# SreenivasVRao/SuperSloMo-VideoInterpolation-PyTorch

Measured on AMD Instinct MI355X. Metric: interpolated 1280x720 frames/sec, higher is better.
Workload: dtype f32

## Files before the change

superslomo-videointerpolation-pytorch_amd/csrc/ssm_wino5.hip:

```cpp
#include "ssm_common.h"
#include "ssm_wino5_pack.h"

#include <atomic>
#include <mutex>
#include <type_traits>
#include <cstdlib>

typedef float f32x4 __attribute__((ext_vector_type(4)));
typedef float f32x2 __attribute__((ext_vector_type(2)));

namespace {

struct W5Params {
    const float *src;
    long long sb, sc;
    int sh;
    int Cin;
    const float *wpk;
    const float *bias;
    float *dst;
    long long dsb, dsc;
    int dsh;
    float *pool;
    long long psb, psc;
    int psh;
    int H, W, Cout;
    int tilesX, tilesY, NB;
    float slope;
    int lrelu;
    int vec;
    const float *add;
    long long asb, asc;
    int ash, adiv;
    unsigned long long *dbg;
};

template <int GTX_, int WTY_, int WTX_>
struct W5Cfg {
    static constexpr int GTX = GTX_, GTY = 16 / GTX_, WTY = WTY_, WTX = WTX_;
    static constexpr int NTX = GTX * WTX, NTY = GTY * WTY, NT = 32;
    static constexpr int TH = 4 * NTY, TW = 4 * NTX;
    static constexpr int CK = 4;
    static constexpr int PH = TH + 4, PW = TW + 8;
    static constexpr int SHIFT = 2;
    static constexpr int NFQ = 16;
    static constexpr int USZ = NFQ * CK * 32 * 4;
    static constexpr int NTP = NT + 2;
    static constexpr int XRW = NTX * 4 + 4;
    static constexpr int VSZ = NFQ * CK * NTP * 4;
    static constexpr int XPL = PH * XRW;
    static constexpr int XSZ = CK * 2 * XPL;
    static constexpr int NDQ = CK * PH * PW / 4, NGP = (NDQ + 63) / 64;
    static constexpr int PCAP = NGP * 256 + 256;
    static constexpr int NGU = USZ / 256, NIU = NGU / 4, NIP = (NGP + 3) / 4;
    static constexpr int NRU = PH * NTX, NRR = (NRU + 63) / 64;
    static constexpr int UOFF = 0, VOFF = 2 * USZ, XOFF = VOFF + VSZ, POFF = XOFF + XSZ;
    static constexpr int BYTES = (POFF + 2 * PCAP) * 4;
    static_assert(WTY * WTX == 2 && (GTX == 4 || GTX == 8 || GTX == 16), "two tile groups of 16 tiles");
    static_assert(PW % 4 == 0 && NGU % 4 == 0, "whole DMA groups");
    static_assert(BYTES <= 160 * 1024, "LDS budget");
};

__device__ __forceinline__ void w5_bt(const float (&e)[8], float (&f)[8]) {
    f[0] = (e[0] - e[6]) + 5.25f * (e[4] - e[2]);
    f[7] = (e[7] - e[1]) + 5.25f * (e[3] - e[5]);
    const float t1 = (e[2] + e[6]) - 4.25f * e[4], t2 = (e[1] + e[5]) - 4.25f * e[3];
    const float t3 = (e[6] + 0.25f * e[2]) - 1.25f * e[4], t4 = (0.5f * e[1] - 2.5f * e[3]) + 2.f * e[5];
    const float t5 = (e[6] + 4.f * e[2]) - 5.f * e[4], t6 = (2.f * e[1] - 2.5f * e[3]) + 0.5f * e[5];
    f[1] = t1 + t2;
    f[2] = t1 - t2;
    f[3] = t3 + t4;
    f[4] = t3 - t4;
    f[5] = t5 + t6;
    f[6] = t5 - t6;
}

__device__ __forceinline__ void w5_at(float m0, float m1, float m2, float m3, float m4, float m5, float m6, float m7, float (&y)[4]) {
    const float s1 = m1 + m2, t1 = m1 - m2, s2 = m3 + m4, t2 = m3 - m4, s3 = m5 + m6, t3 = m5 - m6;
    y[0] = (m0 + s1) + (s2 + s3);
    y[1] = (t1 + 2.f * t2) + 0.5f * t3;
    y[2] = (s1 + 4.f * s2) + 0.25f * s3;
    y[3] = ((t1 + 8.f * t2) + 0.125f * t3) + m7;
}

template <bool FAST>
__device__ __forceinline__ void w5_epilogue(const W5Params &p, const f32x4 (&acc)[64], const float (&bv)[4], int b, int cu0, int q, int px, int py) {
    const float sl = (p.lrelu & 1) ? p.slope : 1.f;
    const bool amask = (p.lrelu & 2) != 0;
    float *dstb = p.dst + (long long)b * p.dsb;
    float *poolb = p.pool ? p.pool + (long long)b * p.psb : nullptr;
    const unsigned pb = 4u * ((unsigned)(4 * q) * (unsigned)p.dsc + (unsigned)py * (unsigned)p.dsh + (unsigned)px);
    const unsigned qb = 4u * ((unsigned)(4 * q) * (unsigned)p.psc + (unsigned)(py >> 1) * (unsigned)p.psh + (unsigned)(px >> 1));
    const bool vok = FAST || (py + 4 <= p.H && px + 4 <= p.W && p.vec);
    auto st4 = [](const float *base, unsigned off_bytes, f32x4 val) {
        asm volatile("global_store_dwordx4 %0, %1, %2" ::"v"(off_bytes), "v"(val), "s"(base) : "memory");
    };
    auto st2 = [](const float *base, unsigned off_bytes, f32x2 val) {
        asm volatile("global_store_dwordx2 %0, %1, %2" ::"v"(off_bytes), "v"(val), "s"(base) : "memory");
    };
    auto st1 = [](const float *base, unsigned off_bytes, float val) {
        asm volatile("global_store_dword %0, %1, %2" ::"v"(off_bytes), "v"(val), "s"(base) : "memory");
    };
    const float *addb = p.add ? p.add + (long long)(b / p.adiv) * p.asb + (long long)(4 * q) * p.asc + (long long)py * p.ash + px : nullptr;
    f32x4 zadd[2][4];
    const bool zvec = p.add && vok;
    auto zload = [&](int r) {
        if (zvec) {
#pragma unroll
            for (int i = 0; i < 4; ++i) zadd[r & 1][i] = *(const f32x4 *)(addb + (long long)(cu0 + r) * p.asc + (long long)i * p.ash);
        }
    };
    zload(0);
#pragma unroll
    for (int r = 0; r < 4; ++r) {
        const int cu = cu0 + r;
        if (r + 1 < 4) zload(r + 1);
        float t[4][8];
#pragma unroll
        for (int cf = 0; cf < 8; ++cf) {
            float y4[4];
            w5_at(acc[cf][r], acc[8 + cf][r], acc[16 + cf][r], acc[24 + cf][r], acc[32 + cf][r], acc[40 + cf][r], acc[48 + cf][r], acc[56 + cf][r], y4);
#pragma unroll
            for (int i = 0; i < 4; ++i) t[i][cf] = y4[i];
        }
        float y[4][4];
#pragma unroll
        for (int i = 0; i < 4; ++i) {
            float y4[4];
            w5_at(t[i][0], t[i][1], t[i][2], t[i][3], t[i][4], t[i][5], t[i][6], t[i][7], y4);
#pragma unroll
            for (int e = 0; e < 4; ++e) y[i][e] = y4[e] + bv[r];
        }
        if (p.add) {
            const float *ap = addb + (long long)cu * p.asc;
#pragma unroll
            for (int i = 0; i < 4; ++i) {
                if (vok) {
                    const f32x4 z = zadd[r & 1][i];
                    if (amask) {
#pragma unroll
                        for (int e = 0; e < 4; ++e) y[i][e] *= z[e] > 0.f ? 1.f : p.slope;
                    } else {
                        y[i][0] += z[0];
                        y[i][1] += z[1];
                        y[i][2] += z[2];
                        y[i][3] += z[3];
                    }
                } else {
#pragma unroll
                    for (int e = 0; e < 4; ++e)
                        if (py + i < p.H && px + e < p.W) {
                                const float z = ap[(long long)i * p.ash + e];
                                y[i][e] = amask ? y[i][e] * (z > 0.f ? 1.f : p.slope) : y[i][e] + z;
                            }
                }
            }
        }
#pragma unroll
        for (int i = 0; i < 4; ++i)
#pragma unroll
            for (int e = 0; e < 4; ++e) y[i][e] = fmaxf(y[i][e], y[i][e] * sl);
        if (zvec && r + 1 < 4) {
#pragma unroll
            for (int i = 0; i < 4; ++i) asm volatile("" : "+v"(zadd[(r + 1) & 1][i]));
        }
        float *bp = dstb + (long long)cu * p.dsc;
#pragma unroll
        for (int i = 0; i < 4; ++i) {
            if (vok) {
                st4(bp + (long long)i * p.dsh, pb, f32x4{y[i][0], y[i][1], y[i][2], y[i][3]});
            } else {
#pragma unroll
                for (int e = 0; e < 4; ++e)
                    if (py + i < p.H && px + e < p.W) st1(bp + (long long)i * p.dsh + e, pb, y[i][e]);
            }
        }
        if (poolb) {
            float *qp = poolb + (long long)cu * p.psc;
#pragma unroll
            for (int i = 0; i < 2; ++i) {
                const float o0 = ((y[2 * i][0] + y[2 * i + 1][0]) + (y[2 * i][1] + y[2 * i + 1][1])) * 0.25f;
                const float o1 = ((y[2 * i][2] + y[2 * i + 1][2]) + (y[2 * i][3] + y[2 * i + 1][3])) * 0.25f;
                const bool rok = FAST || py + 2 * i < p.H;
                if (FAST || (rok && px + 4 <= p.W && p.vec)) st2(qp + (long long)i * p.psh, qb, f32x2{o0, o1});
                else if (rok) {
                    if (px + 2 <= p.W) st1(qp + (long long)i * p.psh, qb, o0);
                    if (px + 4 <= p.W) st1(qp + (long long)i * p.psh + 1, qb, o1);
                }
            }
        }
        __builtin_amdgcn_sched_barrier(0);
    }
}

#if !W5_SPLIT
template <class C>
__global__ __launch_bounds__(256) __attribute__((amdgpu_waves_per_eu(1, 1))) void wino5_kernel(const W5Params p) {
    extern __shared__ __attribute__((aligned(16))) float lds[];
    constexpr int PH = C::PH, PW = C::PW, NTX = C::NTX, CK = C::CK, NFQ = C::NFQ;

    const int tid = threadIdx.x;
    const int lane = tid & 63, l15 = lane & 15, q = lane >> 4;
    const int wid = __builtin_amdgcn_readfirstlane(tid >> 6);
    const int cb = wid & 1, tg = wid >> 1;

    int id = ssm_xcd_tile(blockIdx.x, gridDim.x);
    const int nb = id % p.NB;
    id /= p.NB;
    const int tx = id % p.tilesX;
    id /= p.tilesX;
    const int ty = id % p.tilesY;
    const int b = id / p.tilesY;
    const int x0 = tx * C::TW, y0 = ty * C::TH;

    const float *pbase = p.src + (long long)b * p.sb + (long long)(y0 - 2) * p.sh + (x0 - 4);
    const float *wbase = p.wpk + (long long)nb * (p.Cin / CK) * C::USZ;

    int poff[C::NIP];
#pragma unroll
    for (int i = 0; i < C::NIP; ++i) {
        const int qq = (i * 4 + wid) * 64 + lane;
        if (qq < C::NDQ) {
            const int c = qq / (PH * (PW / 4)), rem = qq - c * (PH * (PW / 4));
            const int r = rem / (PW / 4), j = rem - r * (PW / 4);
            const int re = min(r, p.H + (SSM_PADY - 1) - (y0 - 2)), fe = min(4 * j, ((p.W + 2 * SSM_PADX + 3) & ~3) - 4 - x0);
            poff[i] = ((int)(c * p.sc) + re * p.sh + fe) * 4;
        } else {
            poff[i] = 0;
        }
    }
    const int uoff = lane * 16;
    const unsigned lds0 = (unsigned)(size_t)(__attribute__((address_space(3))) void *)lds;
    auto dma = [](const float *base, int voff_bytes, unsigned m0v) {
        asm volatile("s_mov_b32 m0, %2\n\ts_nop 0\n\tglobal_load_lds_dwordx4 %0, %1" ::"v"(voff_bytes), "s"(base), "s"(m0v) : "memory", "m0");
    };
    auto issue_n = [&](int s, int n) {
        const int buf = s & 1;
        if (n < C::NIP) {
            const int g = 4 * n + wid;
            if (4 * n + 3 < C::NGP || g < C::NGP) {
                const float *base = pbase + (long long)(s * CK) * p.sc;
                const unsigned m0v = __builtin_amdgcn_readfirstlane(lds0 + (unsigned)(C::POFF + buf * C::PCAP + C::SHIFT) * 4u + (unsigned)g * 1024u);
                dma(base, poff[n], m0v);
            }
        } else {
            const int g = 4 * (n - C::NIP) + wid;
            const float *base = wbase + (long long)s * C::USZ + g * 256;
            const unsigned m0v = __builtin_amdgcn_readfirstlane(lds0 + (unsigned)(C::UOFF + buf * C::USZ) * 4u + (unsigned)g * 1024u);
            dma(base, uoff, m0v);
        }
    };
    static_assert(C::NIP + C::NIU <= 16, "one DMA slot per quad of the matrix phase");

    f32x4 acc[64];
#pragma unroll
    for (int f = 0; f < 64; ++f) acc[f] = f32x4{0.f, 0.f, 0.f, 0.f};
    float bv[4];
#pragma unroll
    for (int r = 0; r < 4; ++r) bv[r] = p.bias[nb * 32 + cb * 16 + 4 * q + r];

    int r_src[C::NRR], r_dst[C::NRR];
#pragma unroll
    for (int k = 0; k < C::NRR; ++k) {
        const int u = min(lane + 64 * k, C::NRU - 1);
        const int c = wid, row = u / NTX, t = u - row * NTX;
        r_src[k] = C::POFF + C::SHIFT + (c * PH + row) * PW + 4 * t + 2;
        r_dst[k] = C::XOFF + c * 2 * C::XPL + row * C::XRW + t * 4;
    }
    const int c_tile = lane & 31;
    const int c_gx = (c_tile & 15) % C::GTX, c_gy = (c_tile & 15) / C::GTX, c_g2 = c_tile >> 4;
    const int c_Tx = (c_g2 % C::WTX) * C::GTX + c_gx, c_Ty = (c_g2 / C::WTX) * C::GTY + c_gy;
    const int c_src = C::XOFF + (wid * 2 + (lane >> 5)) * C::XPL + (4 * c_Ty) * C::XRW + c_Tx * 4;
    const int c_dst = C::VOFF + (((lane >> 5) * CK + wid) * C::NTP + c_tile) * 4;

    const f32x4 *lds4 = (const f32x4 *)lds;
    const int aBase = C::UOFF / 4 + q * 32 + cb * 16 + l15;
    const int bBase = C::VOFF / 4 + q * C::NTP + tg * 16 + l15;
    const int gx = l15 % C::GTX, gy = l15 / C::GTX;
    const int Tx = (tg % C::WTX) * C::GTX + gx, Ty = (tg / C::WTX) * C::GTY + gy;

    const int nsteps = p.Cin / CK;
#pragma unroll
    for (int n = 0; n < C::NIP + C::NIU; ++n) issue_n(0, n);
#ifdef W5_TRACE
    unsigned long long tph[6] = {0, 0, 0, 0, 0, 0};
    unsigned long long tk = __builtin_amdgcn_s_memtime();
    const unsigned long long tstart = tk;
#define W5STAMP(i)                                                  \
    {                                                               \
        const unsigned long long tn = __builtin_amdgcn_s_memtime(); \
        tph[i] += tn - tk;                                          \
        tk = tn;                                                    \
    }
#else
#define W5STAMP(i)
#endif
    for (int s = 0; s < nsteps; ++s) {
        const bool more = s + 1 < nsteps;
        W5STAMP(3)
        asm volatile("s_waitcnt vmcnt(0)" ::: "memory");
        __syncthreads();
        W5STAMP(0)
        {
            f32x4 ra[C::NRR][2];
#pragma unroll
            for (int k = 0; k < C::NRR; ++k) {
                const float *src = lds + r_src[k] + (s & 1) * C::PCAP;
                ra[k][0] = *(const f32x4 *)src;
                ra[k][1] = *(const f32x4 *)(src + 4);
            }
#pragma unroll
            for (int k = 0; k < C::NRR; ++k) {
                const float e[8] = {ra[k][0][0], ra[k][0][1], ra[k][0][2], ra[k][0][3], ra[k][1][0], ra[k][1][1], ra[k][1][2], ra[k][1][3]};
                float f[8];
                w5_bt(e, f);
                float *dst = lds + r_dst[k];
                *(f32x4 *)dst = f32x4{f[0], f[1], f[2], f[3]};
                *(f32x4 *)(dst + C::XPL) = f32x4{f[4], f[5], f[6], f[7]};
            }
        }
        W5STAMP(1)
        __builtin_amdgcn_wave_barrier();
        W5STAMP(4)
        {
            f32x4 cx[8];
#pragma unroll
            for (int i = 0; i < 8; ++i) cx[i] = *(const f32x4 *)(lds + c_src + i * C::XRW);
            float f[4][8];
#pragma unroll
            for (int e = 0; e < 4; ++e) {
                float d[8] = {cx[0][e], cx[1][e], cx[2][e], cx[3][e], cx[4][e], cx[5][e], cx[6][e], cx[7][e]};
#pragma unroll
                for (int i = 0; i < 8; ++i) asm volatile("" : "+v"(d[i]));
                w5_bt(d, f[e]);
            }
#pragma unroll
            for (int rf = 0; rf < 8; ++rf) *(f32x4 *)(lds + c_dst + rf * 2 * CK * C::NTP * 4) = f32x4{f[0][rf], f[1][rf], f[2][rf], f[3][rf]};
        }
        W5STAMP(2)
        __syncthreads();
        W5STAMP(5)
        {
            const int ai = aBase + (s & 1) * (C::USZ / 4), bi = bBase;
            f32x4 a[3], bq[3];
            a[0] = lds4[ai];
            bq[0] = lds4[bi];
            a[1] = lds4[ai + CK * 32];
            bq[1] = lds4[bi + CK * C::NTP];
#pragma unroll
            for (int g = 0; g < NFQ; ++g) {
                const int cur = g % 3, nxt = (g + 2) % 3;
#pragma unroll
                for (int e = 0; e < 4; ++e) {
                    acc[4 * g + e] = __builtin_amdgcn_mfma_f32_16x16x4f32(a[cur][e], bq[cur][e], acc[4 * g + e], 0, 0, 0);
                    if (e == 0) {
                        __builtin_amdgcn_sched_barrier(0);
                        if (g + 2 < NFQ) {
                            a[nxt] = lds4[ai + (g + 2) * CK * 32];
                            bq[nxt] = lds4[bi + (g + 2) * CK * C::NTP];
                        }
                        __builtin_amdgcn_sched_barrier(0);
                    }
                    if (e == 1 && g < C::NIP + C::NIU && more) {
                        issue_n(s + 1, g);
                        __builtin_amdgcn_sched_barrier(0);
                    }
                }
                __builtin_amdgcn_sched_barrier(0);
            }
        }
    }
    W5STAMP(3)
    {
        const int px = x0 + 4 * Tx, py = y0 + 4 * Ty;
        w5_epilogue<false>(p, acc, bv, b, nb * 32 + cb * 16, q, px, py);
    }
#ifdef W5_TRACE
    asm volatile("s_waitcnt vmcnt(0)" ::: "memory");
    if (p.dbg && lane == 0 && (blockIdx.x % 64) == 0) {
        const unsigned long long tn = __builtin_amdgcn_s_memtime();
        for (int i = 0; i < 6; ++i) atomicAdd(p.dbg + wid * 8 + i, tph[i]);
        atomicAdd(p.dbg + wid * 8 + 6, tn - tk);
        atomicAdd(p.dbg + wid * 8 + 7, 1ULL);
        (void)tstart;
    }
#endif
}

#endif

#if W5_SPLIT
__device__ __forceinline__ void w5_bt_lo(const float (&e)[8], float (&f)[4]) {
    f[0] = (e[0] - e[6]) + 5.25f * (e[4] - e[2]);
    f[3] = (e[7] - e[1]) + 5.25f * (e[3] - e[5]);
    const float t1 = (e[2] + e[6]) - 4.25f * e[4], t2 = (e[1] + e[5]) - 4.25f * e[3];
    f[1] = t1 + t2;
    f[2] = t1 - t2;
}
__device__ __forceinline__ void w5_bt_hi(const float (&e)[8], float (&f)[4]) {
    const float t3 = (e[6] + 0.25f * e[2]) - 1.25f * e[4], t4 = (0.5f * e[1] - 2.5f * e[3]) + 2.f * e[5];
    const float t5 = (e[6] + 4.f * e[2]) - 5.f * e[4], t6 = (2.f * e[1] - 2.5f * e[3]) + 0.5f * e[5];
    f[0] = t3 + t4;
    f[1] = t3 - t4;
    f[2] = t5 + t6;
    f[3] = t5 - t6;
}

template <class C>
struct W5SLds {
    static constexpr int NPB = 3;
    static constexpr int XRW = C::NTX * 4 + 8, XPL = C::PH * XRW;
    static constexpr int XSZ1 = C::CK * XPL;
    static constexpr int UOFF = 0, VOFF = 2 * C::USZ, XOFF = VOFF + C::VSZ, POFF = XOFF + XSZ1;
    static constexpr int BYTES = (POFF + NPB * C::PCAP) * 4;
    static constexpr int EXSZ = 8 * 2 * 4 * 64 * 4;
    static_assert(BYTES <= 160 * 1024 && EXSZ <= 2 * C::USZ, "LDS budget; the exchange area reuses the filter stages");
};

template <class C>
__global__ __launch_bounds__(512) __attribute__((amdgpu_waves_per_eu(2, 2))) void wino5s_kernel(const W5Params p) {
    extern __shared__ __attribute__((aligned(16))) float lds[];
    using L = W5SLds<C>;
    constexpr int PH = C::PH, PW = C::PW, NTX = C::NTX, CK = C::CK, NTP = C::NTP;

    const int tid = threadIdx.x;
    const int lane = tid & 63, l15 = lane & 15, q = lane >> 4;
    const int wid = __builtin_amdgcn_readfirstlane(tid >> 6);
    const int cb = wid & 1, tg = (wid >> 1) & 1, fh = wid >> 2;
    const int w4 = wid & 3;

    int id = ssm_xcd_tile(blockIdx.x, gridDim.x);
    const int nb = id % p.NB;
    id /= p.NB;
    const int tx = id % p.tilesX;
    id /= p.tilesX;
    const int ty = id % p.tilesY;
    const int b = id / p.tilesY;
    const int x0 = tx * C::TW, y0 = ty * C::TH;

    const float *pbase = p.src + (long long)b * p.sb + (long long)(y0 - 2) * p.sh + (x0 - 4);
    const float *wbase = p.wpk + (long long)nb * (p.Cin / CK) * C::USZ;

    int poff[C::NIP];
#pragma unroll
    for (int i = 0; i < C::NIP; ++i) {
        const int qq = (i * 4 + w4) * 64 + lane;
        if (qq < C::NDQ) {
            const int c = qq / (PH * (PW / 4)), rem = qq - c * (PH * (PW / 4));
            const int r = rem / (PW / 4), j = rem - r * (PW / 4);
            const int re = min(r, p.H + (SSM_PADY - 1) - (y0 - 2)), fe = min(4 * j, ((p.W + 2 * SSM_PADX + 3) & ~3) - 4 - x0);
            poff[i] = ((int)(c * p.sc) + re * p.sh + fe) * 4;
        } else {
            poff[i] = 0;
        }
    }
    const int uoff = lane * 16;
    const unsigned lds0 = (unsigned)(size_t)(__attribute__((address_space(3))) void *)lds;
    auto dma = [](const float *base, int voff_bytes, unsigned m0v) {
        asm volatile("s_mov_b32 m0, %2\n\ts_nop 0\n\tglobal_load_lds_dwordx4 %0, %1" ::"v"(voff_bytes), "s"(base), "s"(m0v) : "memory", "m0");
    };
    struct DmaBase {
        const float *src;
        unsigned m0;
    };
    auto u_base = [&](int s) {
        return DmaBase{wbase + (long long)s * C::USZ + w4 * 256,
                       (unsigned)__builtin_amdgcn_readfirstlane(lds0 + (unsigned)(L::UOFF + (s & 1) * C::USZ) * 4u + (unsigned)w4 * 1024u)};
    };
    auto p_base = [&](int s, int pb) {
        return DmaBase{pbase + (long long)(s * CK) * p.sc,
                       (unsigned)__builtin_amdgcn_readfirstlane(lds0 + (unsigned)(L::POFF + pb * C::PCAP + C::SHIFT) * 4u + (unsigned)w4 * 1024u)};
    };
    auto dma_u = [&](const DmaBase &bs, int k) { dma(bs.src + k * 1024, uoff, bs.m0 + (unsigned)k * 4096u); };
    auto dma_p = [&](const DmaBase &bs, int k) {
        if (4 * k + 3 < C::NGP || 4 * k + w4 < C::NGP) dma(bs.src, poff[k], bs.m0 + (unsigned)k * 4096u);
    };
    static_assert(C::NGU == 32, "8 filter pieces per wave of half 1: the transform's 8 DMA slots");

    f32x4 acc[32];
#pragma unroll
    for (int f = 0; f < 32; ++f) acc[f] = f32x4{0.f, 0.f, 0.f, 0.f};

    int r_src[C::NRR], r_dst[C::NRR];
#pragma unroll
    for (int k = 0; k < C::NRR; ++k) {
        const int u = min(lane + 64 * k, C::NRU - 1);
        const int row = u / NTX, t = u - row * NTX;
        r_src[k] = L::POFF + C::SHIFT + (w4 * PH + row) * PW + 4 * t + 2;
        r_dst[k] = L::XOFF + w4 * L::XPL + row * L::XRW + t * 4;
    }
    const int c_tile = lane >> 1, cp = lane & 1;
    const int c_gx = (c_tile & 15) % C::GTX, c_gy = (c_tile & 15) / C::GTX, c_g2 = c_tile >> 4;
    const int c_Tx = (c_g2 % C::WTX) * C::GTX + c_gx, c_Ty = (c_g2 / C::WTX) * C::GTY + c_gy;
    const int c_src = L::XOFF + w4 * L::XPL + (4 * c_Ty) * L::XRW + c_Tx * 4 + 2 * cp;
    const int c_dst = L::VOFF + ((fh * CK + w4) * NTP + c_tile) * 4 + 2 * cp;

    const f32x4 *lds4 = (const f32x4 *)lds;
    const int aBase = L::UOFF / 4 + fh * (CK * 32) + q * 32 + cb * 16 + l15;
    const int bBase = L::VOFF / 4 + fh * (CK * NTP) + q * NTP + tg * 16 + l15;
    const int gx = l15 % C::GTX, gy = l15 / C::GTX;
    const int Tx = (tg % C::WTX) * C::GTX + gx, Ty = (tg / C::WTX) * C::GTY + gy;

    auto transform = [&](auto FH, int pb, auto slot) __attribute__((always_inline)) {
        constexpr int h = decltype(FH)::value;
        {
            f32x4 ra[C::NRR][2];
#pragma unroll
            for (int k = 0; k < C::NRR; ++k) {
                const float *src = lds + r_src[k] + pb * C::PCAP;
                ra[k][0] = *(const f32x4 *)src;
                ra[k][1] = *(const f32x4 *)(src + 4);
            }
            __builtin_amdgcn_sched_barrier(0);
            slot(0);
            __builtin_amdgcn_sched_barrier(0);
#pragma unroll
            for (int k = 0; k < C::NRR; ++k) {
                const float e[8] = {ra[k][0][0], ra[k][0][1], ra[k][0][2], ra[k][0][3], ra[k][1][0], ra[k][1][1], ra[k][1][2], ra[k][1][3]};
                float f[4];
                if (h == 0) w5_bt_lo(e, f);
                else w5_bt_hi(e, f);
                *(f32x4 *)(lds + r_dst[k]) = f32x4{f[0], f[1], f[2], f[3]};
                __builtin_amdgcn_sched_barrier(0);
                slot(1 + k);
                __builtin_amdgcn_sched_barrier(0);
            }
        }
        __builtin_amdgcn_wave_barrier();
        {
            f32x2 cx[8];
#pragma unroll
            for (int i = 0; i < 8; ++i) cx[i] = *(const f32x2 *)(lds + c_src + i * L::XRW);
            __builtin_amdgcn_sched_barrier(0);
            slot(4);
            __builtin_amdgcn_sched_barrier(0);
            float f[2][8];
#pragma unroll
            for (int e = 0; e < 2; ++e) {
                float d[8] = {cx[0][e], cx[1][e], cx[2][e], cx[3][e], cx[4][e], cx[5][e], cx[6][e], cx[7][e]};
#pragma unroll
                for (int i = 0; i < 8; ++i) asm volatile("" : "+v"(d[i]));
                w5_bt(d, f[e]);
                __builtin_amdgcn_sched_barrier(0);
                slot(5 + e);
                __builtin_amdgcn_sched_barrier(0);
            }
#pragma unroll
            for (int rf = 0; rf < 8; ++rf) *(f32x2 *)(lds + c_dst + rf * 2 * CK * NTP * 4) = f32x2{f[0][rf], f[1][rf]};
            __builtin_amdgcn_sched_barrier(0);
            slot(7);
        }
    };
    static_assert(C::NRR == 3, "DMA slots 1 .. 3 of the transform = the row pass's rounds");

    auto matrix = [&](int st, auto dmaf) __attribute__((always_inline)) {
        const int ai = aBase + st * (C::USZ / 4), bi = bBase;
        f32x4 a[3], bq[3];
        a[0] = lds4[ai];
        bq[0] = lds4[bi];
        a[1] = lds4[ai + 2 * CK * 32];
        bq[1] = lds4[bi + 2 * CK * NTP];
#pragma unroll
        for (int g = 0; g < 8; ++g) {
            const int cur = g % 3, nxt = (g + 2) % 3;
#pragma unroll
            for (int e = 0; e < 4; ++e) {
                acc[4 * g + e] = __builtin_amdgcn_mfma_f32_16x16x4f32(a[cur][e], bq[cur][e], acc[4 * g + e], 0, 0, 0);
                if (e == 0) {
                    __builtin_amdgcn_sched_barrier(0);
                    if (g + 2 < 8) {
                        a[nxt] = lds4[ai + (g + 2) * 2 * CK * 32];
                        bq[nxt] = lds4[bi + (g + 2) * 2 * CK * NTP];
                    }
                    __builtin_amdgcn_sched_barrier(0);
                }
                if (e == 1) {
                    dmaf(g);
                    __builtin_amdgcn_sched_barrier(0);
                }
            }
            __builtin_amdgcn_sched_barrier(0);
        }
    };

#ifdef W5_TRACE
    unsigned long long tph[6] = {0, 0, 0, 0, 0, 0};
    unsigned long long tk = __builtin_amdgcn_s_memtime();
#define W5S(i)                                                      \
    {                                                               \
        const unsigned long long tn = __builtin_amdgcn_s_memtime(); \
        tph[i] += tn - tk;                                          \
        tk = tn;                                                    \
    }
#else
#define W5S(i)
#endif
    const int nsteps = p.Cin / CK;
    if (fh == 0) {
        const DmaBase ub = u_base(0);
#pragma unroll
        for (int k = 0; k < 8; ++k) dma_u(ub, k);
    } else {
        for (int s = 0; s < 3 && s < nsteps; ++s) {
            const DmaBase pbs = p_base(s, s);
#pragma unroll
            for (int k = 0; k < C::NIP; ++k) dma_p(pbs, k);
        }
    }
    asm volatile("s_waitcnt vmcnt(0)" ::: "memory");
    __syncthreads();
    using I0 = std::integral_constant<int, 0>;
    using I1 = std::integral_constant<int, 1>;
    auto noslot = [](int) {};
    if (fh == 0) transform(I0{}, 0, noslot);
    __syncthreads();
    W5S(5)

    const bool first = w4 < C::NGP - 4 * (C::NIP - 1);
    if (fh == 0) {
        int pb1 = 1 % L::NPB;
        for (int s = 0; s < nsteps; ++s) {
            const bool more = s + 1 < nsteps;
            const DmaBase ub = u_base(more ? s + 1 : s);
            matrix(s & 1, [&](int g) {
                if (more) dma_u(ub, g);
            });
            W5S(0)
            __syncthreads();
            W5S(2)
            if (more) transform(I0{}, pb1, noslot);
            pb1 = pb1 + 1 == L::NPB ? 0 : pb1 + 1;
            W5S(1)
            asm volatile("s_waitcnt vmcnt(0)" ::: "memory");
            __syncthreads();
            W5S(3)
        }
    } else {
        int pb = 0;
        for (int s = 0; s < nsteps; ++s) {
            transform(I1{}, pb, noslot);
            W5S(1)
            if (s >= 1 && s + 2 < nsteps) {
                if (first) asm volatile("s_waitcnt vmcnt(%0)" ::"n"(C::NIP) : "memory");
                else asm volatile("s_waitcnt vmcnt(%0)" ::"n"(C::NIP - 1) : "memory");
            } else {
                asm volatile("s_waitcnt vmcnt(0)" ::: "memory");
            }
            __syncthreads();
            W5S(3)
            const bool more3 = s + 3 < nsteps;
            const DmaBase pbs = p_base(more3 ? s + 3 : s, pb);
            matrix(s & 1, [&](int g) {
                if (g < C::NIP && more3) dma_p(pbs, g);
            });
            W5S(0)
            pb = pb + 1 == L::NPB ? 0 : pb + 1;
            __syncthreads();
            W5S(2)
        }
    }

    auto epilogue = [&](auto FHC) __attribute__((always_inline)) {
    constexpr int fh = decltype(FHC)::value;
    auto partial = [&](int r, float (&y)[4][4]) __attribute__((always_inline)) {
        float t[4][4];
#pragma unroll
        for (int e = 0; e < 4; ++e) {
            float y4[4];
            w5_at(acc[e][r], acc[4 + e][r], acc[8 + e][r], acc[12 + e][r], acc[16 + e][r], acc[20 + e][r], acc[24 + e][r], acc[28 + e][r], y4);
#pragma unroll
            for (int i = 0; i < 4; ++i) t[i][e] = y4[i];
        }
#pragma unroll
        for (int i = 0; i < 4; ++i) {
            if (fh == 0) {
                const float s1 = t[i][1] + t[i][2], d1 = t[i][1] - t[i][2];
                y[i][0] = t[i][0] + s1;
                y[i][1] = d1;
                y[i][2] = s1;
                y[i][3] = d1 + t[i][3];
            } else {
                const float s2 = t[i][0] + t[i][1], d2 = t[i][0] - t[i][1], s3 = t[i][2] + t[i][3], d3 = t[i][2] - t[i][3];
                y[i][0] = s2 + s3;
                y[i][1] = 2.f * d2 + 0.5f * d3;
                y[i][2] = 4.f * s2 + 0.25f * s3;
                y[i][3] = 8.f * d2 + 0.125f * d3;
            }
        }
    };
    f32x4 *ex = (f32x4 *)lds;
    {
#pragma unroll
        for (int rr = 0; rr < 2; ++rr) {
            float y[4][4];
            partial(2 * (1 - fh) + rr, y);
#pragma unroll
            for (int i = 0; i < 4; ++i) ex[((wid * 2 + rr) * 4 + i) * 64 + lane] = f32x4{y[i][0], y[i][1], y[i][2], y[i][3]};
        }
    }
    __syncthreads();
    {
        const int px = x0 + 4 * Tx, py = y0 + 4 * Ty;
        const int cu0 = nb * 32 + cb * 16;
        const float sl = (p.lrelu & 1) ? p.slope : 1.f;
    const bool amask = (p.lrelu & 2) != 0;
        float *dstb = p.dst + (long long)b * p.dsb;
        float *poolb = p.pool ? p.pool + (long long)b * p.psb : nullptr;
        const unsigned pbo = 4u * ((unsigned)(4 * q) * (unsigned)p.dsc + (unsigned)py * (unsigned)p.dsh + (unsigned)px);
        const unsigned qbo = 4u * ((unsigned)(4 * q) * (unsigned)p.psc + (unsigned)(py >> 1) * (unsigned)p.psh + (unsigned)(px >> 1));
        const bool vok = py + 4 <= p.H && px + 4 <= p.W && p.vec;
        auto st4 = [](const float *base, unsigned off_bytes, f32x4 val) {
            asm volatile("global_store_dwordx4 %0, %1, %2" ::"v"(off_bytes), "v"(val), "s"(base) : "memory");
        };
        auto st2 = [](const float *base, unsigned off_bytes, f32x2 val) {
            asm volatile("global_store_dwordx2 %0, %1, %2" ::"v"(off_bytes), "v"(val), "s"(base) : "memory");
        };
        auto st1 = [](const float *base, unsigned off_bytes, float val) {
            asm volatile("global_store_dword %0, %1, %2" ::"v"(off_bytes), "v"(val), "s"(base) : "memory");
        };
        const float *addb = p.add ? p.add + (long long)(b / p.adiv) * p.asb + (long long)(4 * q) * p.asc + (long long)py * p.ash + px : nullptr;
#pragma unroll
        for (int rr = 0; rr < 2; ++rr) {
            const int r = 2 * fh + rr;
            const int cu = cu0 + r;
            const float bvr = p.bias[cu + 4 * q];
            float y[4][4];
            partial(r, y);
#pragma unroll
            for (int i = 0; i < 4; ++i) {
                const f32x4 o = ex[(((wid ^ 4) * 2 + rr) * 4 + i) * 64 + lane];
#pragma unroll
                for (int e = 0; e < 4; ++e) y[i][e] = ((fh == 0 ? y[i][e] + o[e] : o[e] + y[i][e])) + bvr;
            }
            if (p.add) {
                const float *ap = addb + (long long)cu * p.asc;
#pragma unroll
                for (int i = 0; i < 4; ++i) {
                    if (vok) {
                        const f32x4 z = *(const f32x4 *)(ap + (long long)i * p.ash);
                        if (amask) {
#pragma unroll
                            for (int e = 0; e < 4; ++e) y[i][e] *= z[e] > 0.f ? 1.f : p.slope;
                        } else {
                            y[i][0] += z[0];
                            y[i][1] += z[1];
                            y[i][2] += z[2];
                            y[i][3] += z[3];
                        }
                    } else {
#pragma unroll
                        for (int e = 0; e < 4; ++e)
                            if (py + i < p.H && px + e < p.W) {
                                const float z = ap[(long long)i * p.ash + e];
                                y[i][e] = amask ? y[i][e] * (z > 0.f ? 1.f : p.slope) : y[i][e] + z;
                            }
                    }
                }
            }
#pragma unroll
            for (int i = 0; i < 4; ++i)
#pragma unroll
                for (int e = 0; e < 4; ++e) y[i][e] = fmaxf(y[i][e], y[i][e] * sl);
            float *bp = dstb + (long long)cu * p.dsc;
#pragma unroll
            for (int i = 0; i < 4; ++i) {
                if (vok) {
                    st4(bp + (long long)i * p.dsh, pbo, f32x4{y[i][0], y[i][1], y[i][2], y[i][3]});
                } else {
#pragma unroll
                    for (int e = 0; e < 4; ++e)
                        if (py + i < p.H && px + e < p.W) st1(bp + (long long)i * p.dsh + e, pbo, y[i][e]);
                }
            }
            if (poolb) {
                float *qp = poolb + (long long)cu * p.psc;
#pragma unroll
                for (int i = 0; i < 2; ++i) {
                    const float o0 = ((y[2 * i][0] + y[2 * i + 1][0]) + (y[2 * i][1] + y[2 * i + 1][1])) * 0.25f;
                    const float o1 = ((y[2 * i][2] + y[2 * i + 1][2]) + (y[2 * i][3] + y[2 * i + 1][3])) * 0.25f;
                    const bool rok = py + 2 * i < p.H;
                    if (rok && px + 4 <= p.W && p.vec) st2(qp + (long long)i * p.psh, qbo, f32x2{o0, o1});
                    else if (rok) {
                        if (px + 2 <= p.W) st1(qp + (long long)i * p.psh, qbo, o0);
                        if (px + 4 <= p.W) st1(qp + (long long)i * p.psh + 1, qbo, o1);
                    }
                }
            }
            __builtin_amdgcn_sched_barrier(0);
        }
    }
    };
    if (fh == 0) epilogue(I0{});
    else epilogue(I1{});
#ifdef W5_TRACE
    asm volatile("s_waitcnt vmcnt(0)" ::: "memory");
    W5S(4)
    if (p.dbg && lane == 0 && (blockIdx.x % 64) == 0) {
        for (int i = 0; i < 6; ++i) atomicAdd(p.dbg + wid * 8 + i, tph[i]);
        atomicAdd(p.dbg + wid * 8 + 7, 1ULL);
    }
#endif
}

#endif

using F5A = W5Cfg<8, 2, 1>;
using F5B = W5Cfg<4, 1, 2>;

#define SSM_W5_KINDS(X) X(F5A_, F5A) X(F5B_, F5B)

enum W5Kind {
#define X(name, cfg) name,
    SSM_W5_KINDS(X)
#undef X
        NW5KIND
};

std::atomic<int> g_force_w5kind{-1};
#ifdef W5_TRACE
std::atomic<unsigned long long *> g_w5dbg{nullptr};
#endif

template <class C>
int w5launch(W5Params &p, int B, hipStream_t st) {
    p.tilesX = (p.W + C::TW - 1) / C::TW;
    p.tilesY = (p.H + C::TH - 1) / C::TH;
    p.NB = p.Cout / 32;
    const long long blocks = (long long)p.tilesX * p.tilesY * p.NB * B;
    if (blocks <= 0 || blocks > 0x7fffffffLL) {
        ssm::set_error("wino5 conv: grid of %lld workgroups out of range", blocks);
        return SSM_E_ARG;
    }
#if W5_SPLIT
    void (*kern)(const W5Params) = wino5s_kernel<C>;
    constexpr int lds_bytes = W5SLds<C>::BYTES, threads = 512;
#else
    void (*kern)(const W5Params) = wino5_kernel<C>;
    constexpr int lds_bytes = C::BYTES, threads = 256;
#endif
    static std::atomic<uint64_t> lds_reserved{0};
    const hipError_t attr_rc = ssm::reserve_lds(lds_reserved, (const void *)kern, lds_bytes);
    if (attr_rc != hipSuccess) {
        ssm::set_error("wino5 conv: cannot reserve %d bytes of LDS: %s", lds_bytes, hipGetErrorString(attr_rc));
        return SSM_E_LAUNCH;
    }
    SSM_LAUNCH(kern, dim3((unsigned)blocks), dim3(threads), lds_bytes, st, p);
    return ssm::check_launch("ssm_wino5_conv2d_add_fwd");
}

int w5dispatch(int kind, W5Params &p, int B, hipStream_t st) {
    switch (kind) {
#define X(name, cfg) \
    case name: return w5launch<cfg>(p, B, st);
        SSM_W5_KINDS(X)
#undef X
    }
    return SSM_E_UNSUPPORTED;
}

__global__ void wino5_pack_kernel(const float *__restrict__ w, const float *__restrict__ bias, float *__restrict__ wp, float *__restrict__ bp,
                                  int Cout, int Cin, int CinP, long long total, int nbias) {
    const long long i = ((long long)blockIdx.x * blockDim.x + threadIdx.x) * 4;
    if (i < total) {
        float out[4];
        auto at = [&](int co, int ci, int ky, int kx) { return w[(((long long)co * Cin + ci) * 5 + ky) * 5 + kx]; };
        ssm_w5_pack_quad(at, Cout, Cin, CinP, i, out);
        *reinterpret_cast<f32x4 *>(wp + i) = f32x4{out[0], out[1], out[2], out[3]};
    }
#pragma unroll
    for (int e = 0; e < 4; ++e)
        if (i + e < nbias) bp[i + e] = (i + e < Cout) ? bias[i + e] : 0.f;
}

}

extern "C" int ssm_wino5_plan(int Cin, int Cout, int B, int H, int W, int *kind) {
    if (Cin <= 0 || Cout <= 0 || Cout % 32) {
        ssm::set_error("wino5 conv: no tile configuration for Cin=%d Cout=%d (Cout a multiple of 32)", Cin, Cout);
        return SSM_E_UNSUPPORTED;
    }
    const int forced = g_force_w5kind.load();
    if (kind) *kind = (forced >= 0 && forced < NW5KIND) ? forced : 0;
    return SSM_OK;
}

#ifdef W5_TRACE
extern "C" int ssm_wino5_debug_buffer(unsigned long long *dev_counters) {
    g_w5dbg.store(dev_counters);
    return SSM_OK;
}
#endif

extern "C" int ssm_wino5_force_kind(int kind) {
    g_force_w5kind.store(kind >= 0 && kind < NW5KIND ? kind : -1);
    return NW5KIND;
}

extern "C" size_t ssm_wino5_packed_weight_floats(int Cout, int CinP) { return (size_t)(Cout / 32) * (size_t)(CinP / 4) * 16 * 4 * 32 * 4; }

extern "C" int ssm_wino5_pack_weights(const float *w, const float *bias, float *wp, float *bp, int Cout, int Cin, int CinP, void *stream) {
    SSM_REQUIRE(w && bias && wp && bp, "wino5 pack_weights: null pointer");
    SSM_REQUIRE(Cout > 0 && Cin > 0 && Cout % 32 == 0 && CinP >= Cin && CinP % 4 == 0, "wino5 pack_weights: bad sizes (Cout a multiple of 32, CinP of 4)");
    SSM_REQUIRE(ssm::aligned16(wp), "wino5 pack_weights: the packed filter must be 16-byte aligned");
    const long long total = (long long)ssm_wino5_packed_weight_floats(Cout, CinP);
    const int nbias = Cout;
    const long long n = (total > nbias ? total : nbias) / 4 + 1;
    SSM_LAUNCH(wino5_pack_kernel, dim3((unsigned)((n + 255) / 256)), dim3(256), 0, (hipStream_t)stream, w, bias, wp, bp, Cout, Cin, CinP,
                       total, nbias);
    return ssm::check_launch("ssm_wino5_pack_weights");
}

extern "C" int ssm_wino5_conv2d_add_fwd(ssm_view x, int Cin, const float *w_packed, const float *bias_packed, ssm_view y, ssm_view pool,
                                        ssm_view add, int add_div, int B, int H, int W, int Cout, float slope, int flags, void *stream) {
    int kind = 0;
    SSM_REQUIRE(B > 0 && H > 0 && W > 0 && Cout > 0 && Cin > 0, "wino5 conv: bad sizes");
    const int rc = ssm_wino5_plan(Cin, Cout, B, H, W, &kind);
    if (rc != SSM_OK) return rc;
    SSM_REQUIRE(x.ptr && y.ptr && w_packed && bias_packed, "wino5 conv: null pointer");
    SSM_REQUIRE(Cin % 4 == 0, "wino5 conv: the channel count (%d) must be a multiple of 4 (pad the view)", Cin);
    SSM_REQUIRE(ssm::aligned16(x.ptr) && x.sh % 4 == 0 && x.sc % 4 == 0 && x.sb % 4 == 0,
                "wino5 conv: the input is not a padded-plane view (16-byte alignment)");
    SSM_REQUIRE(x.sh >= W + 2 * SSM_PADX, "wino5 conv: input row stride %d leaves no zero frame for W=%d", x.sh, W);
    SSM_REQUIRE(ssm::aligned16(w_packed), "wino5 conv: packed filter must be 16-byte aligned");
    SSM_REQUIRE(4LL * x.sc * 4 < 0x7fffffffLL, "wino5 conv: channel stride too large");
    W5Params p;
    p.src = x.ptr;
    p.sb = x.sb;
    p.sc = x.sc;
    p.sh = x.sh;
    p.Cin = Cin;
    p.wpk = w_packed;
    p.bias = bias_packed;
    p.dst = y.ptr;
    p.dsb = y.sb;
    p.dsc = y.sc;
    p.dsh = y.sh;
    p.pool = nullptr;
    p.psb = p.psc = 0;
    p.psh = 0;
    p.H = H;
    p.W = W;
    p.Cout = Cout;
    p.slope = slope;
    p.lrelu = ((flags & SSM_FLAG_LRELU) ? 1 : 0) | ((flags & SSM_FLAG_MASK) ? 2 : 0);
    p.add = nullptr;
    p.asb = p.asc = 0;
    p.ash = 0;
    p.adiv = 1;
    bool vec = W % 4 == 0 && ssm::aligned16(y.ptr) && y.sh % 4 == 0 && y.sc % 4 == 0 && y.sb % 4 == 0;
    if (add.ptr) {
        SSM_REQUIRE(add_div >= 1 && B % add_div == 0, "wino5 conv: the addend serves %d batch entries each, batch %d is no multiple", add_div, B);
        p.add = add.ptr;
        p.asb = add.sb;
        p.asc = add.sc;
        p.ash = add.sh;
        p.adiv = add_div;
        vec = vec && ssm::aligned16(add.ptr) && add.sh % 4 == 0 && add.sc % 4 == 0 && add.sb % 4 == 0;
    }
    if (pool.ptr) {
        SSM_REQUIRE(H % 2 == 0 && W % 2 == 0, "wino5 conv: fused pool needs even H, W");
        p.pool = pool.ptr;
        p.psb = pool.sb;
        p.psc = pool.sc;
        p.psh = pool.sh;
        vec = vec && (reinterpret_cast<size_t>(pool.ptr) & 7) == 0 && pool.sh % 2 == 0 && pool.sc % 2 == 0 && pool.sb % 2 == 0;
    }
    p.vec = vec ? 1 : 0;
#ifdef W5_TRACE
    p.dbg = g_w5dbg.load();
#else
    p.dbg = nullptr;
#endif
    return w5dispatch(kind, p, B, (hipStream_t)stream);
}
```

Baseline: 399.9.

## Balance Winograd input-transform row pass between wave halves by interleaving into matrix loop

Adds a balanced mode to the split 5x5 Winograd kernel, on by default through W5_RM=1. Each wave half now does part of the next step's row transform (RM rows) inside its matrix loop, interleaved with the MFMA groups. To support this it double-buffers the X staging area per filter half, packs the X rows tightly with a small pad every four rows, and reorders the barriers and waits on the fh=1 side. The goal is to hide transform latency behind matrix work and even out the load between the two halves, at the cost of more LDS and extra register pressure during the matrix loop.

```diff
diff --git a/superslomo-videointerpolation-pytorch_amd/csrc/ssm_wino5.hip b/superslomo-videointerpolation-pytorch_amd/csrc/ssm_wino5.hip
--- a/superslomo-videointerpolation-pytorch_amd/csrc/ssm_wino5.hip
+++ b/superslomo-videointerpolation-pytorch_amd/csrc/ssm_wino5.hip
@@ -406,22 +406,35 @@
     f[3] = t5 - t6;
 }
 
-template <class C>
+#ifndef W5_RM
+#define W5_RM 1
+#endif
+
+template <class C, bool BAL = false>
 struct W5SLds {
     static constexpr int NPB = 3;
-    static constexpr int XRW = C::NTX * 4 + 8, XPL = C::PH * XRW;
+    static constexpr int XRW = C::NTX * 4 + 8;
+    static constexpr int XR = C::NTX * 4;
+    __host__ __device__ static constexpr int xr(int r) { return BAL ? XR * r + 32 * (r >> 2) : r * XRW; }
+    static constexpr int XPL = BAL ? xr(C::PH - 1) + XR : C::PH * XRW;
     static constexpr int XSZ1 = C::CK * XPL;
-    static constexpr int UOFF = 0, VOFF = 2 * C::USZ, XOFF = VOFF + C::VSZ, POFF = XOFF + XSZ1;
-    static constexpr int BYTES = (POFF + NPB * C::PCAP) * 4;
+    static constexpr int NXS = BAL ? 2 : 1;
+    static constexpr int NTP = BAL ? C::NT : C::NTP;
+    static constexpr int VSZ = C::NFQ * C::CK * NTP * 4;
+    static constexpr int PCAP = BAL ? (C::NGP * 256 + C::SHIFT + 3) / 4 * 4 : C::PCAP;
+    static constexpr int UOFF = 0, VOFF = 2 * C::USZ, XOFF = VOFF + VSZ, POFF = XOFF + NXS * XSZ1;
+    static constexpr int BYTES = (POFF + NPB * PCAP) * 4;
     static constexpr int EXSZ = 8 * 2 * 4 * 64 * 4;
     static_assert(BYTES <= 160 * 1024 && EXSZ <= 2 * C::USZ, "LDS budget; the exchange area reuses the filter stages");
+    static_assert(!BAL || (C::NTX == 8 && (POFF + C::SHIFT) % 4 == 2 && PCAP % 4 == 0), "BAL: 32-float X rows, 16-byte aligned patch windows");
 };
 
-template <class C>
+template <class C, int RM>
 __global__ __launch_bounds__(512) __attribute__((amdgpu_waves_per_eu(2, 2))) void wino5s_kernel(const W5Params p) {
     extern __shared__ __attribute__((aligned(16))) float lds[];
-    using L = W5SLds<C>;
-    constexpr int PH = C::PH, PW = C::PW, NTX = C::NTX, CK = C::CK, NTP = C::NTP;
+    constexpr bool BAL = RM > 0;
+    using L = W5SLds<C, BAL>;
+    constexpr int PH = C::PH, PW = C::PW, NTX = C::NTX, CK = C::CK, NTP = L::NTP;
 
     const int tid = threadIdx.x;
     const int lane = tid & 63, l15 = lane & 15, q = lane >> 4;
@@ -469,7 +482,7 @@
     };
     auto p_base = [&](int s, int pb) {
         return DmaBase{pbase + (long long)(s * CK) * p.sc,
-                       (unsigned)__builtin_amdgcn_readfirstlane(lds0 + (unsigned)(L::POFF + pb * C::PCAP + C::SHIFT) * 4u + (unsigned)w4 * 1024u)};
+                       (unsigned)__builtin_amdgcn_readfirstlane(lds0 + (unsigned)(L::POFF + pb * L::PCAP + C::SHIFT) * 4u + (unsigned)w4 * 1024u)};
     };
     auto dma_u = [&](const DmaBase &bs, int k) { dma(bs.src + k * 1024, uoff, bs.m0 + (unsigned)k * 4096u); };
     auto dma_p = [&](const DmaBase &bs, int k) {
@@ -487,12 +500,12 @@
         const int u = min(lane + 64 * k, C::NRU - 1);
         const int row = u / NTX, t = u - row * NTX;
         r_src[k] = L::POFF + C::SHIFT + (w4 * PH + row) * PW + 4 * t + 2;
-        r_dst[k] = L::XOFF + w4 * L::XPL + row * L::XRW + t * 4;
+        r_dst[k] = L::XOFF + (BAL ? fh * CK + w4 : w4) * L::XPL + L::xr(row) + t * 4;
     }
     const int c_tile = lane >> 1, cp = lane & 1;
     const int c_gx = (c_tile & 15) % C::GTX, c_gy = (c_tile & 15) / C::GTX, c_g2 = c_tile >> 4;
     const int c_Tx = (c_g2 % C::WTX) * C::GTX + c_gx, c_Ty = (c_g2 / C::WTX) * C::GTY + c_gy;
-    const int c_src = L::XOFF + w4 * L::XPL + (4 * c_Ty) * L::XRW + c_Tx * 4 + 2 * cp;
+    const int c_src = L::XOFF + (BAL ? fh * CK + w4 : w4) * L::XPL + L::xr(4 * c_Ty) + c_Tx * 4 + 2 * cp;
     const int c_dst = L::VOFF + ((fh * CK + w4) * NTP + c_tile) * 4 + 2 * cp;
 
     const f32x4 *lds4 = (const f32x4 *)lds;
@@ -501,26 +514,31 @@
     const int gx = l15 % C::GTX, gy = l15 / C::GTX;
     const int Tx = (tg % C::WTX) * C::GTX + gx, Ty = (tg / C::WTX) * C::GTY + gy;
 
-    auto transform = [&](auto FH, int pb, auto slot) __attribute__((always_inline)) {
+    auto row_read = [&](int k, int pb, f32x4 (&ra)[2]) __attribute__((always_inline)) {
+        const float *src = lds + r_src[k] + pb * L::PCAP;
+        ra[0] = *(const f32x4 *)src;
+        ra[1] = *(const f32x4 *)(src + 4);
+    };
+    auto row_write = [&](auto FH, int k, const f32x4 (&ra)[2]) __attribute__((always_inline)) {
         constexpr int h = decltype(FH)::value;
-        {
+        const float e[8] = {ra[0][0], ra[0][1], ra[0][2], ra[0][3], ra[1][0], ra[1][1], ra[1][2], ra[1][3]};
+        float f[4];
+        if (h == 0) w5_bt_lo(e, f);
+        else w5_bt_hi(e, f);
+        *(f32x4 *)(lds + r_dst[k]) = f32x4{f[0], f[1], f[2], f[3]};
+    };
+    auto transform = [&](auto FH, auto K0, int pb, auto slot) __attribute__((always_inline)) {
+        constexpr int k0 = decltype(K0)::value;
+        if constexpr (k0 < C::NRR) {
             f32x4 ra[C::NRR][2];
 #pragma unroll
-            for (int k = 0; k < C::NRR; ++k) {
-                const float *src = lds + r_src[k] + pb * C::PCAP;
-                ra[k][0] = *(const f32x4 *)src;
-                ra[k][1] = *(const f32x4 *)(src + 4);
-            }
+            for (int k = k0; k < C::NRR; ++k) row_read(k, pb, ra[k]);
             __builtin_amdgcn_sched_barrier(0);
             slot(0);
             __builtin_amdgcn_sched_barrier(0);
 #pragma unroll
-            for (int k = 0; k < C::NRR; ++k) {
-                const float e[8] = {ra[k][0][0], ra[k][0][1], ra[k][0][2], ra[k][0][3], ra[k][1][0], ra[k][1][1], ra[k][1][2], ra[k][1][3]};
-                float f[4];
-                if (h == 0) w5_bt_lo(e, f);
-                else w5_bt_hi(e, f);
-                *(f32x4 *)(lds + r_dst[k]) = f32x4{f[0], f[1], f[2], f[3]};
+            for (int k = k0; k < C::NRR; ++k) {
+                row_write(FH, k, ra[k]);
                 __builtin_amdgcn_sched_barrier(0);
                 slot(1 + k);
                 __builtin_amdgcn_sched_barrier(0);
@@ -530,7 +548,7 @@
         {
             f32x2 cx[8];
 #pragma unroll
-            for (int i = 0; i < 8; ++i) cx[i] = *(const f32x2 *)(lds + c_src + i * L::XRW);
+            for (int i = 0; i < 8; ++i) cx[i] = *(const f32x2 *)(lds + c_src + L::xr(i));
             __builtin_amdgcn_sched_barrier(0);
             slot(4);
             __builtin_amdgcn_sched_barrier(0);
@@ -553,7 +571,7 @@
     };
     static_assert(C::NRR == 3, "DMA slots 1 .. 3 of the transform = the row pass's rounds");
 
-    auto matrix = [&](int st, auto dmaf) __attribute__((always_inline)) {
+    auto matrix = [&](int st, auto dmaf, auto rowf) __attribute__((always_inline)) {
         const int ai = aBase + st * (C::USZ / 4), bi = bBase;
         f32x4 a[3], bq[3];
         a[0] = lds4[ai];
@@ -578,10 +596,23 @@
                     dmaf(g);
                     __builtin_amdgcn_sched_barrier(0);
                 }
+                if (BAL && e == 2) {
+                    rowf(g);
+                    __builtin_amdgcn_sched_barrier(0);
+                }
             }
             __builtin_amdgcn_sched_barrier(0);
         }
     };
+    f32x4 rm_ra[2];
+    auto row_share = [&](auto FH, int pb, int g) __attribute__((always_inline)) {
+#pragma unroll
+        for (int k = 0; k < RM; ++k) {
+            if (g == 2 * k) row_read(k, pb, rm_ra);
+            if (g == 2 * k + 1) row_write(FH, k, rm_ra);
+        }
+    };
+    auto norow = [](int) {};
 
 #ifdef W5_TRACE
     unsigned long long tph[6] = {0, 0, 0, 0, 0, 0};
@@ -611,12 +642,14 @@
     __syncthreads();
     using I0 = std::integral_constant<int, 0>;
     using I1 = std::integral_constant<int, 1>;
+    using IRM = std::integral_constant<int, RM>;
     auto noslot = [](int) {};
-    if (fh == 0) transform(I0{}, 0, noslot);
+    const bool first = w4 < C::NGP - 4 * (C::NIP - 1);
+    if constexpr (!BAL) {
+    if (fh == 0) transform(I0{}, I0{}, 0, noslot);
     __syncthreads();
     W5S(5)
 
-    const bool first = w4 < C::NGP - 4 * (C::NIP - 1);
     if (fh == 0) {
         int pb1 = 1 % L::NPB;
         for (int s = 0; s < nsteps; ++s) {
@@ -624,11 +657,11 @@
             const DmaBase ub = u_base(more ? s + 1 : s);
             matrix(s & 1, [&](int g) {
                 if (more) dma_u(ub, g);
-            });
+            }, norow);
             W5S(0)
             __syncthreads();
             W5S(2)
-            if (more) transform(I0{}, pb1, noslot);
+            if (more) transform(I0{}, I0{}, pb1, noslot);
             pb1 = pb1 + 1 == L::NPB ? 0 : pb1 + 1;
             W5S(1)
             asm volatile("s_waitcnt vmcnt(0)" ::: "memory");
@@ -638,7 +671,7 @@
     } else {
         int pb = 0;
         for (int s = 0; s < nsteps; ++s) {
-            transform(I1{}, pb, noslot);
+            transform(I1{}, I0{}, pb, noslot);
             W5S(1)
             if (s >= 1 && s + 2 < nsteps) {
                 if (first) asm volatile("s_waitcnt vmcnt(%0)" ::"n"(C::NIP) : "memory");
@@ -652,7 +685,7 @@
             const DmaBase pbs = p_base(more3 ? s + 3 : s, pb);
             matrix(s & 1, [&](int g) {
                 if (g < C::NIP && more3) dma_p(pbs, g);
-            });
+            }, norow);
             W5S(0)
             pb = pb + 1 == L::NPB ? 0 : pb + 1;
             __syncthreads();
@@ -660,6 +693,67 @@
         }
     }
 
+    } else {
+    if (fh == 0) {
+        transform(I0{}, I0{}, 0, noslot);
+    } else {
+#pragma unroll
+        for (int k = 0; k < RM; ++k) {
+            row_read(k, 0, rm_ra);
+            row_write(I1{}, k, rm_ra);
+        }
+    }
+    __syncthreads();
+    W5S(5)
+
+    if (fh == 0) {
+        int pb1 = 1 % L::NPB;
+        for (int s = 0; s < nsteps; ++s) {
+            const bool more = s + 1 < nsteps;
+            const DmaBase ub = u_base(more ? s + 1 : s);
+            matrix(s & 1, [&](int g) {
+                if (more) dma_u(ub, g);
+            }, [&](int g) {
+                if (more) row_share(I0{}, pb1, g);
+            });
+            W5S(0)
+            __syncthreads();
+            W5S(2)
+            if (more) transform(I0{}, IRM{}, pb1, noslot);
+            pb1 = pb1 + 1 == L::NPB ? 0 : pb1 + 1;
+            W5S(1)
+            asm volatile("s_waitcnt vmcnt(0)" ::: "memory");
+            __syncthreads();
+            W5S(3)
+        }
+    } else {
+        int pb = 0;
+        for (int s = 0; s < nsteps; ++s) {
+            transform(I1{}, IRM{}, pb, noslot);
+            W5S(1)
+            __syncthreads();
+            W5S(3)
+            const bool more3 = s + 3 < nsteps, more = s + 1 < nsteps;
+            const int pbn = pb + 1 == L::NPB ? 0 : pb + 1;
+            const DmaBase pbs = p_base(more3 ? s + 3 : s, pb);
+            matrix(s & 1, [&](int g) {
+                if (g < C::NIP && more3) dma_p(pbs, g);
+            }, [&](int g) {
+                if (more) row_share(I1{}, pbn, g);
+            });
+            W5S(0)
+            pb = pbn;
+            if (more3) {
+                if (first) asm volatile("s_waitcnt vmcnt(%0)" ::"n"(C::NIP) : "memory");
+                else asm volatile("s_waitcnt vmcnt(%0)" ::"n"(C::NIP - 1) : "memory");
+            } else {
+                asm volatile("s_waitcnt vmcnt(0)" ::: "memory");
+            }
+            __syncthreads();
+            W5S(2)
+        }
+    }
+    }
     auto epilogue = [&](auto FHC) __attribute__((always_inline)) {
     constexpr int fh = decltype(FHC)::value;
     auto partial = [&](int r, float (&y)[4][4]) __attribute__((always_inline)) {
@@ -821,6 +915,18 @@
 std::atomic<unsigned long long *> g_w5dbg{nullptr};
 #endif
 
+template <void (*KERN)(const W5Params), int LDS_BYTES, int THREADS>
+int w5launch_kern(W5Params &p, long long blocks, hipStream_t st) {
+    static std::atomic<uint64_t> lds_reserved{0};
+    const hipError_t attr_rc = ssm::reserve_lds(lds_reserved, (const void *)KERN, LDS_BYTES);
+    if (attr_rc != hipSuccess) {
+        ssm::set_error("wino5 conv: cannot reserve %d bytes of LDS: %s", LDS_BYTES, hipGetErrorString(attr_rc));
+        return SSM_E_LAUNCH;
+    }
+    SSM_LAUNCH(KERN, dim3((unsigned)blocks), dim3(THREADS), LDS_BYTES, st, p);
+    return ssm::check_launch("ssm_wino5_conv2d_add_fwd");
+}
+
 template <class C>
 int w5launch(W5Params &p, int B, hipStream_t st) {
     p.tilesX = (p.W + C::TW - 1) / C::TW;
@@ -832,20 +938,17 @@
         return SSM_E_ARG;
     }
 #if W5_SPLIT
-    void (*kern)(const W5Params) = wino5s_kernel<C>;
-    constexpr int lds_bytes = W5SLds<C>::BYTES, threads = 512;
+    const char *env = getenv("SSM_WINO5_BALANCE");
+    const int rm = env && *env >= '0' && *env <= '3' && env[1] == 0 ? *env - '0' : W5_RM;
+    switch (rm) {
+    case 0: return w5launch_kern<wino5s_kernel<C, 0>, W5SLds<C, false>::BYTES, 512>(p, blocks, st);
+    case 1: return w5launch_kern<wino5s_kernel<C, 1>, W5SLds<C, true>::BYTES, 512>(p, blocks, st);
+    case 2: return w5launch_kern<wino5s_kernel<C, 2>, W5SLds<C, true>::BYTES, 512>(p, blocks, st);
+    default: return w5launch_kern<wino5s_kernel<C, 3>, W5SLds<C, true>::BYTES, 512>(p, blocks, st);
+    }
 #else
-    void (*kern)(const W5Params) = wino5_kernel<C>;
-    constexpr int lds_bytes = C::BYTES, threads = 256;
+    return w5launch_kern<wino5_kernel<C>, C::BYTES, 256>(p, blocks, st);
 #endif
-    static std::atomic<uint64_t> lds_reserved{0};
-    const hipError_t attr_rc = ssm::reserve_lds(lds_reserved, (const void *)kern, lds_bytes);
-    if (attr_rc != hipSuccess) {
-        ssm::set_error("wino5 conv: cannot reserve %d bytes of LDS: %s", lds_bytes, hipGetErrorString(attr_rc));
-        return SSM_E_LAUNCH;
-    }
-    SSM_LAUNCH(kern, dim3((unsigned)blocks), dim3(threads), lds_bytes, st, p);
-    return ssm::check_launch("ssm_wino5_conv2d_add_fwd");
 }
 
 int w5dispatch(int kind, W5Params &p, int B, hipStream_t st) {
```

New measurement: 400.8 (median of 5 runs). Within noise of the previous version (+0.2%).
